# snap-research/F8Net

Hardware: AMD Instinct MI355X
Metric: images/sec at bs=128 (ResNet-50 INT8) (higher is better)
Workload: dtype int8 x int8 -> int32 (exact integer)

## Files before the change

f8net_amd/csrc/f8_cchain.hip:

```cpp
#include "f8_device.h"
#include <algorithm>
#include <cstdio>
#include <cstdlib>

namespace f8 {

struct CCfg {
    static constexpr int C = 2048, MID = 512, PXI = 49, IMG = 4, NPX = PXI * IMG, NPT = 7, G = 8;
    static constexpr int CT = C / 32, CM = MID / 32, CTC = CT / G, CMC = CM / G;
    static constexpr int NK1 = C / 32, KK = MID / 32;
    static constexpr int X8_BYTES = NPT * NK1 * 1024, M_BYTES = NPT * KK * 1024;
    static constexpr int OFF_M1 = X8_BYTES, OFF_M2 = X8_BYTES + M_BYTES, XCL_BYTES = X8_BYTES + 2 * M_BYTES;
    static constexpr int PATCH_BYTES = M_BYTES;
    static constexpr int ZERO_BYTES = 8192;
    static constexpr int D1 = 3, CH1_FR = 40, CH1_BYTES = CH1_FR * 1024;
    static constexpr int D2 = 4, CH2_BYTES = 8 * 1024;
    static constexpr int OFF_ZERO = PATCH_BYTES, OFF_RING2 = PATCH_BYTES + ZERO_BYTES;
    static constexpr int OFF_BIAS = OFF_RING2 + D2 * CH2_BYTES, BIAS_INTS = 32 * (2 * CMC + CTC);
    static constexpr int OFF_MISC = OFF_BIAS + BIAS_INTS * 4, LDS_BYTES = OFF_MISC + 256;
    static_assert(D1 * CH1_BYTES <= OFF_RING2, "the P1 ring lives in the patch's bytes (dead during P1)");
    static_assert(LDS_BYTES <= 160 * 1024, "LDS");
};
constexpr size_t kCChainXchgBytes = (size_t)32 * CCfg::XCL_BYTES;

template <int FAST>
__device__ __forceinline__ v4i cq_tile16(const v16i& y, int n, int lo, int hi, unsigned x_or) {
    unsigned d[4];
    const float sc = FAST == 1 ? requant_u8_scale(n) : 0.0f;
#pragma unroll
    for (int g = 0; g < 4; ++g) {
        if constexpr (FAST == 1) d[g] = requant_u8x4(y[4 * g], y[4 * g + 1], y[4 * g + 2], y[4 * g + 3], sc) ^ x_or;
        else if constexpr (FAST == 2) d[g] = requant_u8x4_int(y[4 * g], y[4 * g + 1], y[4 * g + 2], y[4 * g + 3], n) ^ x_or;
        else d[g] = pack4(requant1(y[4 * g], n, lo, hi), requant1(y[4 * g + 1], n, lo, hi), requant1(y[4 * g + 2], n, lo, hi), requant1(y[4 * g + 3], n, lo, hi)) ^ x_or;
    }
    auto s0 = __builtin_amdgcn_permlane32_swap(d[0], d[2], false, false);
    auto s1 = __builtin_amdgcn_permlane32_swap(d[1], d[3], false, false);
    const v4i o = {(int)s0[0], (int)s0[1], (int)s1[0], (int)s1[1]};
    return o;
}

#define F8_LDS3(p) ((__attribute__((address_space(3))) void*)(p))

#ifndef F8_CC_Q_TAIL
#define F8_CC_Q_TAIL 0
#endif
#ifndef F8_CC_Q_P1
#define F8_CC_Q_P1 0
#endif
#ifndef F8_CC_Q_P2
#define F8_CC_Q_P2 0
#endif
#ifndef F8_CC_Q_P3
#define F8_CC_Q_P3 0
#endif
#define F8_CC_QI(fast, ov) ((fast) == 1 && (ov) != 0 ? (ov) : (fast))

#ifndef F8_CC_WAR_NOPS
#define F8_CC_WAR_NOPS 16
#endif
__device__ __forceinline__ void mfma_operands_read() {
#ifdef F8_CC_NO_GUARD
    return;
#endif
    __builtin_amdgcn_sched_barrier(0);
    if constexpr (F8_CC_WAR_NOPS >= 16) asm volatile("s_nop 7\n\ts_nop 7" ::: "memory");
    else if constexpr (F8_CC_WAR_NOPS >= 8) asm volatile("s_nop 7" ::: "memory");
    else if constexpr (F8_CC_WAR_NOPS >= 4) asm volatile("s_nop 3" ::: "memory");
    else if constexpr (F8_CC_WAR_NOPS >= 2) asm volatile("s_nop 1" ::: "memory");
    else if constexpr (F8_CC_WAR_NOPS >= 1) asm volatile("s_nop 0" ::: "memory");
    __builtin_amdgcn_sched_barrier(0);
}

__device__ __forceinline__ void lds_barrier() {
    asm volatile("s_waitcnt lgkmcnt(0)" ::: "memory");
    __builtin_amdgcn_s_barrier();
    asm volatile("" ::: "memory");
}

template <int FAST>
__global__ void __launch_bounds__(512) __attribute__((amdgpu_waves_per_eu(2, 2)))
cchain_kernel(const ChainArgs a) {
    using Cfg = CCfg;
    constexpr int C = Cfg::C, NPT = Cfg::NPT, NK1 = Cfg::NK1, KK = Cfg::KK;
#ifndef F8_CC_DBG_NOSETREG
    if constexpr (FAST == 1) set_fp_round_nearest_even();
#endif
    extern __shared__ __attribute__((aligned(16))) char lds[];
    char* const ring2 = lds + Cfg::OFF_RING2;
    int* const bias_lds = (int*)(lds + Cfg::OFF_BIAS);
    int* const misc = (int*)(lds + Cfg::OFF_MISC);

    const int tid = threadIdx.x;
    const int wave = __builtin_amdgcn_readfirstlane(tid >> 6) & 7;
    const int lane = tid & 63, l31 = lane & 31, lh = lane >> 5;
    const unsigned l16 = (unsigned)(lane * 16);
    const int pp = wave & 3, kh = wave >> 2;

    if (tid == 0) misc[0] = (int)__hip_atomic_fetch_add(a.sync, 1u, __ATOMIC_RELAXED, __HIP_MEMORY_SCOPE_AGENT);
    __syncthreads();
    const int L = __builtin_amdgcn_readfirstlane(misc[0]);
    const int cl = L >> 3, c = L & 7;
    const int ncl = (int)(gridDim.x >> 3);
    const int ngroups = (a.N + Cfg::IMG - 1) / Cfg::IMG;
    const int npix = a.N * Cfg::PXI;
    unsigned* const flags = a.sync + 16;
    const unsigned long long t_limit = (unsigned long long)a.timeout_ticks;
    unsigned seq = 0;
#ifdef F8_TRACE
    unsigned tt[12] = {}; unsigned t_prev = (unsigned)__builtin_readcyclecounter();
#define F8_CT(i) do { const unsigned now_ = (unsigned)__builtin_readcyclecounter(); tt[i] += now_ - t_prev; t_prev = now_; } while (0)
#else
#define F8_CT(i)
#endif

    const __amdgpu_buffer_rsrc_t rxc = __builtin_amdgcn_make_buffer_rsrc((void*)(a.xchg + (size_t)cl * Cfg::XCL_BYTES), 0, (unsigned)Cfg::XCL_BYTES, 0x00020000);
    auto wrsrc = [](const int8_t* p) { return __builtin_amdgcn_make_buffer_rsrc((void*)p, 0, 0x7ffffff0, 0x00020000); };

    auto publish = [&]() {
        ++seq;
        asm volatile("s_waitcnt vmcnt(0)" ::: "memory");
        __syncthreads();
        if (tid == 0) __hip_atomic_store(flags + L, seq, __ATOMIC_RELAXED, __HIP_MEMORY_SCOPE_AGENT);
    };
    auto wait_all = [&]() {
        if (tid < Cfg::G && tid != c) {
            unsigned* const f = flags + cl * Cfg::G + tid;
            const unsigned long long t0 = wall_clock64();
            bool ok = true;
            while ((int)(__hip_atomic_load(f, __ATOMIC_RELAXED, __HIP_MEMORY_SCOPE_AGENT) - seq) < 0) {
                __builtin_amdgcn_s_sleep(1);
                if (wall_clock64() - t0 > t_limit) { ok = false; break; }
                if ((__hip_atomic_load(a.err, __ATOMIC_RELAXED, __HIP_MEMORY_SCOPE_AGENT) >> 8) == a.epoch) break;
            }
            if (!ok) {
                __hip_atomic_store(a.err, (a.epoch << 8) | 0x80u | ((unsigned)seq & 0x3fu), __ATOMIC_RELAXED, __HIP_MEMORY_SCOPE_AGENT);
                if (a.err_host) __hip_atomic_store(a.err_host, (a.epoch << 8) | 0x80u | ((unsigned)seq & 0x3fu), __ATOMIC_RELAXED, __HIP_MEMORY_SCOPE_SYSTEM);
            }
        }
        __syncthreads();
    };
    auto load_patch = [&](int off) {
#pragma unroll
        for (int k = 0; k < 14; ++k) {
            const int e = wave * 14 + k;
            __builtin_amdgcn_raw_ptr_buffer_load_lds(rxc, F8_LDS3(lds + e * 1024), 16, l16, off + e * 1024, 0, 17);
        }
    };

    v16i res[NPT];
    const int ct = c * Cfg::CTC + wave;

    for (int grp = cl; grp < ngroups; grp += ncl) {
        const int m0 = grp * Cfg::NPX;
        if (a.tail) {
            const ChainBlk& B = a.blk[0];
            const bool sc_first = B.res_shl == 0;
            const __amdgpu_buffer_rsrc_t rxs = __builtin_amdgcn_make_buffer_rsrc((void*)a.x8in, 0, (unsigned)(a.N * 196 * 1024), 0x00020000);
            const __amdgpu_buffer_rsrc_t rm2 = __builtin_amdgcn_make_buffer_rsrc((void*)a.m2in, 0, (unsigned)(npix * 512), 0x00020000);
            const __amdgpu_buffer_rsrc_t rwsc = wrsrc(B.wsc), rw4 = wrsrc(B.w4);
            unsigned vx, vm;
            {
                const int p = wave * 32 + l31, m = m0 + p;
                const int pi = p / Cfg::PXI, rem = p - pi * Cfg::PXI, r = rem / 7, cc = rem - r * 7;
                const bool ok = wave < NPT && p < Cfg::NPX && m < npix;
                vx = ok ? (unsigned)((((grp * Cfg::IMG + pi) * 14 + 2 * r) * 14 + 2 * cc) * 1024 + lh * 16) : kOOB;
                vm = ok ? (unsigned)(m * 512 + lh * 16) : kOOB;
            }
            auto chunk_is_sc = [&](int cq) { return sc_first ? cq < 4 : cq >= 2; };
            auto chunk_k = [&](int cq) { return sc_first ? (cq < 4 ? cq : cq - 4) : (cq < 2 ? cq : cq - 2); };
            auto issue = [&](int cq) {
                char* const buf = lds + (cq & 1) * 65536 + wave * 8192;
                const bool sc = chunk_is_sc(cq);
                const int k0 = chunk_k(cq) * 256;
#pragma unroll
                for (int st = 0; st < 8; ++st) {
                    if (sc) __builtin_amdgcn_raw_ptr_buffer_load_lds(rxs, F8_LDS3(buf + st * 1024), 16, vx, k0 + st * 32, 0, 0);
                    else __builtin_amdgcn_raw_ptr_buffer_load_lds(rm2, F8_LDS3(buf + st * 1024), 16, vm, k0 + st * 32, 0, 0);
                }
            };
            v4i wa[2][8];
            auto load_w = [&](v4i (&dst)[8], int cq) {
                const bool sc = chunk_is_sc(cq);
                const int f0 = (ct * (sc ? 32 : 16) + chunk_k(cq) * 8) * 1024;
#pragma unroll
                for (int st = 0; st < 8; ++st) dst[st] = sc ? __builtin_amdgcn_raw_buffer_load_b128(rwsc, l16, f0 + st * 1024, 0) : __builtin_amdgcn_raw_buffer_load_b128(rw4, l16, f0 + st * 1024, 0);
            };
            issue(0);
            load_w(wa[0], 0);
            {
                const int32_t* const bf = sc_first ? B.bsc : B.b4;
#pragma unroll
                for (int g = 0; g < 4; ++g) {
                    const v4i bv = *(const v4i*)(bf + ct * 32 + 8 * g + 4 * lh);
#pragma unroll
                    for (int j = 0; j < NPT; ++j)
#pragma unroll
                        for (int e = 0; e < 4; ++e) res[j][4 * g + e] = bv[e];
                }
            }
            static_for<6>([&](auto qc) {
                constexpr int Q = decltype(qc)::value;
                asm volatile("s_waitcnt vmcnt(0)" ::: "memory");
                lds_barrier();
                if constexpr (Q + 1 < 6) { issue(Q + 1); load_w(wa[(Q + 1) & 1], Q + 1); }
                const char* const buf = lds + (Q & 1) * 65536;
#pragma unroll
                for (int st = 0; st < 8; ++st)
#pragma unroll
                    for (int j = 0; j < NPT; ++j) {
                        const v4i xf = *(const v4i*)(buf + (j * 8 + st) * 1024 + l16);
                        res[j] = __builtin_amdgcn_mfma_i32_32x32x32_i8(wa[Q & 1][st], xf, res[j], 0, 0, 0);
                    }
                mfma_operands_read();
                if ((sc_first && Q == 3) || (!sc_first && Q == 1)) {
                    const int sh = sc_first ? B.acc_shl : B.res_shl;
                    const int32_t* const bs = sc_first ? B.b4 : B.bsc;
#pragma unroll
                    for (int g = 0; g < 4; ++g) {
                        const v4i bv = *(const v4i*)(bs + ct * 32 + 8 * g + 4 * lh);
#pragma unroll
                        for (int j = 0; j < NPT; ++j)
#pragma unroll
                            for (int e = 0; e < 4; ++e) res[j][4 * g + e] = (int)(((unsigned)res[j][4 * g + e] << sh) + (unsigned)bv[e]);
                    }
                }
            });
            const int floor1 = B.relu1 ? 0 : -2147483647;
            const ChainBlk& B1 = a.blk[1];
#pragma unroll
            for (int j = 0; j < NPT; ++j) {
#pragma unroll
                for (int r = 0; r < 16; ++r) res[j][r] = max(res[j][r], floor1);
                const v4i o = cq_tile16<F8_CC_QI(FAST, F8_CC_Q_TAIL)>(res[j], B1.nq, FAST ? 0 : B1.loq, FAST ? 255 : B1.hiq, FAST ? 0x80808080u : B1.xorq);
                __builtin_amdgcn_raw_buffer_store_b128(o, rxc, l16, (j * NK1 + ct) * 1024, 17);
            }
            publish();
            F8_CT(0);
        } else {
            const ChainBlk& B0 = a.blk[0];
            const __amdgpu_buffer_rsrc_t rxr = __builtin_amdgcn_make_buffer_rsrc((void*)a.xr, 0, (unsigned)(((npix + 31) & ~31) * C * 4), 0x00020000);
#pragma unroll
            for (int j = 0; j < NPT; ++j) {
                const int p = j * 32 + l31, m = m0 + p;
                const unsigned vo = (p < Cfg::NPX && m < npix) ? (unsigned)((m >> 5) * (C * 128) + lh * 512 + (m & 31) * 16) : kOOB;
#pragma unroll
                for (int g = 0; g < 4; ++g) {
                    const v4i v = __builtin_amdgcn_raw_buffer_load_b128(rxr, vo + g * 1024, ct * 4096, 0);
#pragma unroll
                    for (int e = 0; e < 4; ++e) res[j][4 * g + e] = v[e];
                }
            }
#pragma unroll
            for (int j = 0; j < NPT; ++j) {
                const v4i o = cq_tile16<FAST>(res[j], B0.nq, FAST ? 0 : B0.loq, FAST ? 255 : B0.hiq, FAST ? 0x80808080u : B0.xorq);
                __builtin_amdgcn_raw_buffer_store_b128(o, rxc, l16, (j * NK1 + ct) * 1024, 17);
            }
            publish();
            F8_CT(0);
        }

        for (int b = a.tail ? 1 : 0; b < a.nblk; ++b) {
            const ChainBlk& B = a.blk[b];
            const bool last = b + 1 == a.nblk;
            const ChainBlk& BN = a.blk[last ? b : b + 1];
            const int n1 = B.n1, n2 = B.n2, acc_shl = B.acc_shl, res_shl = B.res_shl;
            const int lo1 = FAST ? 0 : B.lo1, hi1 = FAST ? 255 : B.hi1, lo2 = FAST ? 0 : B.lo2, hi2 = FAST ? 255 : B.hi2;
            const unsigned xor1 = FAST ? 0x80808080u : B.xor1, xor2 = FAST ? 0x80808080u : B.xor2;
            const int relu_a = FAST ? 1 : B.relu_a, relu_b = FAST ? 1 : B.relu_b, relu1 = FAST ? 1 : B.relu1;
            const int nq = BN.nq, loq = FAST ? 0 : BN.loq, hiq = FAST ? 255 : BN.hiq;
            const unsigned xorq = FAST ? 0x80808080u : BN.xorq;

            {
                int bv = 0;
                if (tid < 64) bv = B.b0[c * 64 + tid];
                else if (tid < 128) bv = B.b2[c * 64 + tid - 64];
                else if (tid < Cfg::BIAS_INTS) bv = B.b4[c * 256 + tid - 128];
                if (tid < Cfg::BIAS_INTS) bias_lds[tid] = bv;
            }
            wait_all();
            F8_CT(1);

            {
                const __amdgpu_buffer_rsrc_t rw0 = wrsrc(B.w0);
                v16i acc[2][2];
#pragma unroll
                for (int jj = 0; jj < 2; ++jj)
#pragma unroll
                    for (int i = 0; i < 2; ++i)
#pragma unroll
                        for (int r = 0; r < 16; ++r) acc[jj][i][r] = 0;
                constexpr int NCH = NK1 / 4, D = Cfg::D1, NI = 5;
                auto issue = [&](int q) {
                    char* const slot = lds + (q % D) * Cfg::CH1_BYTES;
#pragma unroll
                    for (int k = 0; k < NI; ++k) {
                        const int e = wave * NI + k, t = e & 3;
                        const int step = t < 2 ? 2 * q + t : 32 + 2 * q + (t - 2);
                        if (e < 32) {
                            const int j = e >> 2;
                            __builtin_amdgcn_raw_ptr_buffer_load_lds(rxc, F8_LDS3(slot + e * 1024), 16, j < NPT ? l16 : kOOB, (j * NK1 + step) * 1024, 0, 17);
                        } else {
                            const int i = (e - 32) >> 2;
                            __builtin_amdgcn_raw_ptr_buffer_load_lds(rw0, F8_LDS3(slot + e * 1024), 16, l16, ((c * 2 + i) * NK1 + step) * 1024, 0, 0);
                        }
                    }
                };
                asm volatile("s_waitcnt vmcnt(0)" ::: "memory");
                issue(0); issue(1);
                const unsigned bb = (unsigned)((pp * 8 + kh * 2) * 1024) + l16, ab = (unsigned)((32 + kh * 2) * 1024) + l16;
                static_for<NCH>([&](auto qc) {
                    constexpr int Q = decltype(qc)::value;
                    constexpr int younger = (Q + D - 2 < NCH - 1 ? Q + D - 2 : NCH - 1) - Q;
                    wait_vmcnt<younger * NI>();
                    lds_barrier();
                    if constexpr (Q + D - 1 < NCH) issue(Q + D - 1);
                    const char* const slot = lds + (Q % D) * Cfg::CH1_BYTES;
#pragma unroll
                    for (int s = 0; s < 2; ++s) {
                        const v4i a0 = *(const v4i*)(slot + ab + s * 1024), a1 = *(const v4i*)(slot + ab + (4 + s) * 1024);
                        const v4i b0 = *(const v4i*)(slot + bb + s * 1024), b1 = *(const v4i*)(slot + bb + (4 + s) * 1024);
                        acc[0][0] = __builtin_amdgcn_mfma_i32_32x32x32_i8(a0, b0, acc[0][0], 0, 0, 0);
                        acc[0][1] = __builtin_amdgcn_mfma_i32_32x32x32_i8(a1, b0, acc[0][1], 0, 0, 0);
                        acc[1][0] = __builtin_amdgcn_mfma_i32_32x32x32_i8(a0, b1, acc[1][0], 0, 0, 0);
                        acc[1][1] = __builtin_amdgcn_mfma_i32_32x32x32_i8(a1, b1, acc[1][1], 0, 0, 0);
                    }
                });
                mfma_operands_read();
                F8_CT(2);
                __syncthreads();
#pragma unroll
                for (int jj = 0; jj < 2; ++jj)
#pragma unroll
                    for (int g = 0; g < 4; ++g) {
                        v4i o;
#pragma unroll
                        for (int e = 0; e < 4; ++e) o[e] = kh ? acc[jj][0][4 * g + e] : acc[jj][1][4 * g + e];
                        *(v4i*)(lds + (wave * 8 + jj * 4 + g) * 1024 + l16) = o;
                    }
                __syncthreads();
                const int floor0 = relu_a ? 0 : INT32_MIN;
                const int ctm = c * 2 + kh;
#pragma unroll
                for (int jj = 0; jj < 2; ++jj) {
                    v16i y;
#pragma unroll
                    for (int g = 0; g < 4; ++g) {
                        const v4i o = *(const v4i*)(lds + ((wave ^ 4) * 8 + jj * 4 + g) * 1024 + l16);
                        const v4i bv = *(const v4i*)(bias_lds + kh * 32 + 8 * g + 4 * lh);
#pragma unroll
                        for (int e = 0; e < 4; ++e) {
                            const unsigned mine = (unsigned)(kh ? acc[jj][1][4 * g + e] : acc[jj][0][4 * g + e]);
                            y[4 * g + e] = (int)(mine + (unsigned)o[e] + (unsigned)bv[e]);
                            if constexpr (!FAST) y[4 * g + e] = max(y[4 * g + e], floor0);
                        }
                    }
                    const int j = pp * 2 + jj;
                    const v4i o = cq_tile16<F8_CC_QI(FAST, F8_CC_Q_P1)>(y, n1, lo1, hi1, xor1);
                    if (j < NPT) __builtin_amdgcn_raw_buffer_store_b128(o, rxc, l16, Cfg::OFF_M1 + (j * KK + ctm) * 1024, 17);
                }
                publish();
                F8_CT(3);
            }
            {
                const v4i zv = {(int)xor1, (int)xor1, (int)xor1, (int)xor1};
                *(v4i*)(lds + Cfg::OFF_ZERO + tid * 16) = zv;
            }
            wait_all();
            F8_CT(4);

            {
                const __amdgpu_buffer_rsrc_t rw2 = wrsrc(B.w2);
                load_patch(Cfg::OFF_M1);
                constexpr int NCH = 36, D = Cfg::D2;
                auto issue = [&](int q) {
                    const int e = wave, i = e >> 2, t = e & 3;
                    const int step = (q >> 2) * KK + (t < 2 ? 0 : 8) + 2 * (q & 3) + (t & 1);
                    __builtin_amdgcn_raw_ptr_buffer_load_lds(rw2, F8_LDS3(ring2 + (q % D) * Cfg::CH2_BYTES + e * 1024), 16, l16, ((c * 2 + i) * (9 * KK) + step) * 1024, 0, 0);
                };
                issue(0); issue(1); issue(2);
                int prow[2], pcol[2];
#pragma unroll
                for (int jj = 0; jj < 2; ++jj) {
                    const int p = (pp * 2 + jj) * 32 + l31;
                    const int rem = p % Cfg::PXI, r = rem / 7;
                    prow[jj] = p < Cfg::NPX ? r : 64; pcol[jj] = rem - r * 7;
                }
                unsigned tb[2] = {0u, 0u};
                auto tap_base = [&](auto tc) {
                    constexpr int T = decltype(tc)::value, TY = T / 3 - 1, TX = T % 3 - 1;
#pragma unroll
                    for (int jj = 0; jj < 2; ++jj) {
                        const int q = (pp * 2 + jj) * 32 + l31 + TY * 7 + TX;
                        const bool ok = (unsigned)(prow[jj] + TY) < 7u && (unsigned)(pcol[jj] + TX) < 7u;
                        tb[jj] = ok ? (unsigned)((q >> 5) * (KK * 1024) + kh * 8192 + lh * 512 + (q & 31) * 16) : (unsigned)Cfg::OFF_ZERO + l16;
                    }
                };
                v16i acc[2][2];
#pragma unroll
                for (int jj = 0; jj < 2; ++jj)
#pragma unroll
                    for (int i = 0; i < 2; ++i)
#pragma unroll
                        for (int r = 0; r < 16; ++r) acc[jj][i][r] = 0;
                const unsigned ab = (unsigned)(kh * 2 * 1024) + l16;
                static_for<NCH>([&](auto qc) {
                    constexpr int Q = decltype(qc)::value, T = Q / 4;
                    constexpr int younger = (Q + D - 2 < NCH - 1 ? Q + D - 2 : NCH - 1) - Q;
                    wait_vmcnt<younger>();
                    lds_barrier();
                    if constexpr (Q + D - 1 < NCH) issue(Q + D - 1);
                    if constexpr (Q % 4 == 0) tap_base(std::integral_constant<int, T>{});
                    const char* const slot = ring2 + (Q % D) * Cfg::CH2_BYTES;
#pragma unroll
                    for (int s = 0; s < 2; ++s) {
                        const v4i a0 = *(const v4i*)(slot + ab + s * 1024), a1 = *(const v4i*)(slot + ab + (4 + s) * 1024);
                        const v4i b0 = *(const v4i*)(lds + tb[0] + (2 * (Q % 4) + s) * 1024), b1 = *(const v4i*)(lds + tb[1] + (2 * (Q % 4) + s) * 1024);
                        acc[0][0] = __builtin_amdgcn_mfma_i32_32x32x32_i8(a0, b0, acc[0][0], 0, 0, 0);
                        acc[0][1] = __builtin_amdgcn_mfma_i32_32x32x32_i8(a1, b0, acc[0][1], 0, 0, 0);
                        acc[1][0] = __builtin_amdgcn_mfma_i32_32x32x32_i8(a0, b1, acc[1][0], 0, 0, 0);
                        acc[1][1] = __builtin_amdgcn_mfma_i32_32x32x32_i8(a1, b1, acc[1][1], 0, 0, 0);
                    }
                });
                mfma_operands_read();
                F8_CT(5);
                __syncthreads();
#pragma unroll
                for (int jj = 0; jj < 2; ++jj)
#pragma unroll
                    for (int g = 0; g < 4; ++g) {
                        v4i o;
#pragma unroll
                        for (int e = 0; e < 4; ++e) o[e] = kh ? acc[jj][0][4 * g + e] : acc[jj][1][4 * g + e];
                        *(v4i*)(lds + (wave * 8 + jj * 4 + g) * 1024 + l16) = o;
                    }
                __syncthreads();
                const int floor0 = relu_b ? 0 : INT32_MIN;
                const int ctm = c * 2 + kh;
#pragma unroll
                for (int jj = 0; jj < 2; ++jj) {
                    v16i y;
#pragma unroll
                    for (int g = 0; g < 4; ++g) {
                        const v4i o = *(const v4i*)(lds + ((wave ^ 4) * 8 + jj * 4 + g) * 1024 + l16);
                        const v4i bv = *(const v4i*)(bias_lds + 64 + kh * 32 + 8 * g + 4 * lh);
#pragma unroll
                        for (int e = 0; e < 4; ++e) {
                            const unsigned mine = (unsigned)(kh ? acc[jj][1][4 * g + e] : acc[jj][0][4 * g + e]);
                            y[4 * g + e] = (int)(mine + (unsigned)o[e] + (unsigned)bv[e]);
                            if constexpr (!FAST) y[4 * g + e] = max(y[4 * g + e], floor0);
                        }
                    }
                    const int j = pp * 2 + jj;
                    const v4i o = cq_tile16<F8_CC_QI(FAST, F8_CC_Q_P2)>(y, n2, lo2, hi2, xor2);
                    if (j < NPT) __builtin_amdgcn_raw_buffer_store_b128(o, rxc, l16, Cfg::OFF_M2 + (j * KK + ctm) * 1024, 17);
                }
                publish();
                F8_CT(6);
            }

            {
                const __amdgpu_buffer_rsrc_t rw4 = wrsrc(B.w4);
                v4i wst[KK];
#pragma unroll
                for (int k = 0; k < KK; ++k) wst[k] = __builtin_amdgcn_raw_buffer_load_b128(rw4, l16, (ct * KK + k) * 1024, 0);
                v16i breg;
#pragma unroll
                for (int g = 0; g < 4; ++g) {
                    const v4i bv = *(const v4i*)(bias_lds + 128 + wave * 32 + 8 * g + 4 * lh);
#pragma unroll
                    for (int e = 0; e < 4; ++e) breg[4 * g + e] = bv[e];
                }
                wait_all();
                F8_CT(7);
                load_patch(Cfg::OFF_M2);
                asm volatile("s_waitcnt vmcnt(0)" ::: "memory");
                __syncthreads();
                F8_CT(8);
                const int floor1 = relu1 ? 0 : -2147483647;
                static_for<NPT>([&](auto jc) {
                    constexpr int J = decltype(jc)::value;
                    v16i acc;
#pragma unroll
                    for (int k = 0; k < KK; ++k) {
                        const v4i xf = *(const v4i*)(lds + (J * KK + k) * 1024 + l16);
                        if (k == 0) acc = __builtin_amdgcn_mfma_i32_32x32x32_i8(wst[k], xf, breg, 0, 0, 0);
                        else acc = __builtin_amdgcn_mfma_i32_32x32x32_i8(wst[k], xf, acc, 0, 0, 0);
                    }
                    mfma_operands_read();
                    v16i& rr = res[J];
#pragma unroll
                    for (int r = 0; r < 16; ++r) {
                        if constexpr (FAST) rr[r] = max((int)(((unsigned)acc[r] << acc_shl) + (unsigned)rr[r]), 0);
                        else rr[r] = max((int)(((unsigned)acc[r] << acc_shl) + ((unsigned)rr[r] << res_shl)), floor1);
                    }
                    if (!last) {
                        const v4i o = cq_tile16<F8_CC_QI(FAST, F8_CC_Q_P3)>(rr, nq, loq, hiq, xorq);
                        __builtin_amdgcn_raw_buffer_store_b128(o, rxc, l16, (J * NK1 + ct) * 1024, 17);
                    } else if (!a.pool) {
                        const int p = J * 32 + l31, m = m0 + p;
                        if (p < Cfg::NPX && m < npix) {
                            const unsigned tot = (unsigned)(((npix + 31) & ~31) * C);
                            if (a.out32) {
                                const __amdgpu_buffer_rsrc_t ro = __builtin_amdgcn_make_buffer_rsrc((void*)a.out32, 0, tot * 4u, 0x00020000);
                                const unsigned vo = (unsigned)((m >> 5) * (C * 128) + lh * 512 + (m & 31) * 16);
#pragma unroll
                                for (int g = 0; g < 4; ++g) {
                                    const v4i o = {rr[4 * g], rr[4 * g + 1], rr[4 * g + 2], rr[4 * g + 3]};
                                    __builtin_amdgcn_raw_buffer_store_b128(o, ro, vo + g * 1024, ct * 4096, 0);
                                }
                            }
#pragma unroll
                            for (int k = 0; k < 2; ++k)
                                if (a.q[k].ptr) {
                                    const __amdgpu_buffer_rsrc_t rq = __builtin_amdgcn_make_buffer_rsrc((void*)a.q[k].ptr, 0, tot, 0x00020000);
                                    __builtin_amdgcn_raw_buffer_store_b128(cq_tile16<0>(rr, a.q[k].n, a.q[k].lo, a.q[k].hi, a.q[k].bias_xor), rq, (unsigned)(m * C + 16 * lh), ct * 32, 0);
                                }
                        }
                    }
                });
                if (last && a.pool) {
                    const bool b0 = lane & 1, b1 = lane & 2;
                    const int n_img = grp * Cfg::IMG + (lane & 3);
#pragma unroll
                    for (int g = 0; g < 4; ++g) {
                        unsigned tot[4];
#pragma unroll
                        for (int e = 0; e < 4; ++e) {
                            unsigned sm[Cfg::IMG];
                            static_for<Cfg::IMG>([&](auto ic) {
                                constexpr int I = decltype(ic)::value, LO = I * Cfg::PXI, HI = LO + Cfg::PXI;
                                unsigned acc_i = 0;
                                static_for<NPT>([&](auto jc) {
                                    constexpr int J = decltype(jc)::value;
                                    if constexpr (J * 32 < HI && J * 32 + 32 > LO) {
                                        constexpr int L0 = LO - J * 32, L1 = HI - J * 32;
                                        acc_i += (l31 >= L0 && l31 < L1) ? (unsigned)res[J][4 * g + e] : 0u;
                                    }
                                });
                                sm[I] = acc_i;
                            });
                            const unsigned u0 = (b0 ? sm[1] : sm[0]) + (unsigned)__shfl_xor((int)(b0 ? sm[0] : sm[1]), 1);
                            const unsigned u1 = (b0 ? sm[3] : sm[2]) + (unsigned)__shfl_xor((int)(b0 ? sm[2] : sm[3]), 1);
                            unsigned v = (b1 ? u1 : u0) + (unsigned)__shfl_xor((int)(b1 ? u0 : u1), 2);
                            v += (unsigned)__shfl_xor((int)v, 4); v += (unsigned)__shfl_xor((int)v, 8); v += (unsigned)__shfl_xor((int)v, 16);
                            tot[e] = v;
                        }
                        if (l31 < Cfg::IMG && n_img < a.N) {
                            const int ch = ct * 32 + 8 * g + 4 * lh;
                            if (a.out32) { const v4i o = {(int)tot[0], (int)tot[1], (int)tot[2], (int)tot[3]}; *(v4i*)(a.out32 + i32t_index(n_img, ch, C)) = o; }
#pragma unroll
                            for (int k = 0; k < 2; ++k)
                                if (a.q[k].ptr)
                                    *(unsigned*)(a.q[k].ptr + (size_t)n_img * C + ch) =
                                        pack4(requant1((int)tot[0], a.q[k].n, a.q[k].lo, a.q[k].hi), requant1((int)tot[1], a.q[k].n, a.q[k].lo, a.q[k].hi),
                                              requant1((int)tot[2], a.q[k].n, a.q[k].lo, a.q[k].hi), requant1((int)tot[3], a.q[k].n, a.q[k].lo, a.q[k].hi)) ^ a.q[k].bias_xor;
                        }
                    }
                }
                F8_CT(9);
                if (!last) publish();
                else __syncthreads();
                F8_CT(10);
            }
        }
    }
    if (tid == 0) {
        asm volatile("s_waitcnt vmcnt(0)" ::: "memory");
        misc[2] = (__hip_atomic_fetch_add(a.sync + 1, 1u, __ATOMIC_RELAXED, __HIP_MEMORY_SCOPE_AGENT) == gridDim.x - 1u) ? 1 : 0;
    }
    __syncthreads();
    if (misc[2]) {
        for (int i = tid; i < (int)gridDim.x; i += 512) __hip_atomic_store(flags + i, 0u, __ATOMIC_RELAXED, __HIP_MEMORY_SCOPE_AGENT);
        if (tid == 0) { __hip_atomic_store(a.sync, 0u, __ATOMIC_RELAXED, __HIP_MEMORY_SCOPE_AGENT); __hip_atomic_store(a.sync + 1, 0u, __ATOMIC_RELAXED, __HIP_MEMORY_SCOPE_AGENT); }
    }
#ifdef F8_TRACE
    if (a.trace && lane == 0) {
        unsigned* tp = (unsigned*)a.trace + ((size_t)blockIdx.x * 8 + wave) * 16;
        for (int i = 0; i < 12; ++i) tp[i] = tt[i];
        tp[12] = (unsigned)L;
    }
#endif
}

bool cchain_supported(int C, int MID, int H, int W, int cin0, bool tail) { return C == 2048 && MID == 512 && H == 7 && W == 7 && cin0 == (tail ? 1024 : 2048); }
size_t cchain_xchg_bytes() { return kCChainXchgBytes; }
int cchain_clusters(int N, int slots) {
    const int groups = (N + CCfg::IMG - 1) / CCfg::IMG, cap = std::min(slots / CCfg::G, 32);
    if (cap < 1) return 0;
    const int rounds = (groups + cap - 1) / cap;
    return (groups + rounds - 1) / rounds;
}
int cchain_kernel_name(char* buf, size_t cap, int fast) { return snprintf(buf, cap, "f8::cchain_kernel<%d>", fast != 0 ? 2 : 0); }

template <int FAST>
static hipError_t launch_cchain_t(const ChainArgs& a, hipStream_t s) {
    static unsigned long long attr_done = 0; int attr_dev = -1;
    if (!dyn_lds_opted_in(&attr_done, &attr_dev)) {
        hipError_t e = hipFuncSetAttribute((const void*)cchain_kernel<FAST>, hipFuncAttributeMaxDynamicSharedMemorySize, CCfg::LDS_BYTES);
        if (e != hipSuccess) return e;
        if (attr_dev >= 0) attr_done |= 1ull << attr_dev;
    }
    const int grid = a.NG * CCfg::G;
    if (a.NG < 1 || grid > 256 || (a.tail ? (!a.x8in || !a.m2in || a.nblk < 2) : !a.xr)) return hipErrorInvalidValue;
#ifdef F8_TRACE
    static unsigned* tbuf = nullptr; static int count = 0;
    static const int want = [] { const char* e = getenv("F8_TRACE_CHAIN7"); return e ? atoi(e) : -1; }();
    ChainArgs b = a;
    const bool tracing = (count++ == want);
    if (tracing) { if (!tbuf) (void)hipMalloc((void**)&tbuf, (size_t)256 * 8 * 64); (void)hipMemsetAsync(tbuf, 0, (size_t)grid * 8 * 64, s); b.trace = tbuf; }
    hipLaunchKernelGGL((cchain_kernel<FAST>), dim3(grid), dim3(512), CCfg::LDS_BYTES, s, b);
    if (tracing) {
        (void)hipStreamSynchronize(s);
        static unsigned hb[256 * 8 * 16];
        (void)hipMemcpy(hb, tbuf, (size_t)grid * 8 * 64, hipMemcpyDeviceToHost);
        static const char* nm[11] = {"stage-in+publish", "wait x8", "P1 loop", "P1 epilogue+publish", "wait mid1", "P2 loop", "P2 epilogue+publish", "wait mid2", "P3 patch load", "P3 compute", "P3 publish"};
        for (int w : {0, 3, 4, 7}) {
            double ph[12] = {};
            for (int i = 0; i < grid; ++i) for (int k = 0; k < 12; ++k) ph[k] += (double)hb[((size_t)i * 8 + w) * 16 + k];
            fprintf(stderr, "[trace cchain<%d>] grid %d, %d blocks, N %d, wave %d: avg cycles per WG (whole launch):", FAST, grid, a.nblk, a.N, w);
            double tot = 0;
            for (int k = 0; k < 11; ++k) { fprintf(stderr, " %s %.0f |", nm[k], ph[k] / grid); tot += ph[k] / grid; }
            fprintf(stderr, " total %.0f\n", tot);
        }
    }
#else
    hipLaunchKernelGGL((cchain_kernel<FAST>), dim3(grid), dim3(512), CCfg::LDS_BYTES, s, a);
#endif
    return hipGetLastError();
}

hipError_t launch_cchain(const ChainArgs& a, int fast, hipStream_t s) {
#ifdef F8_CC_FLOAT_INSTANCE
    if (fast == 1) return launch_cchain_t<1>(a, s);
#endif
    return fast != 0 ? launch_cchain_t<2>(a, s) : launch_cchain_t<0>(a, s);
}

}
```

Measured before the change: 156,800.

## Deepen tail-phase LDS ring to four smaller chunks with two-ahead prefetch

The tail (downsample+conv3) phase now splits its K loop into 12 chunks of 128 instead of 6 chunks of 256. It uses a 4-deep LDS ring, issues loads two chunks ahead and waits with a partial vmcnt instead of draining all loads each step. Separately, lane and offset values are rematerialised per phase behind opaque asm barriers. This stops the compiler hoisting them into long-lived registers and keeps scalar offset bases out of VGPRs, easing register pressure. The cost is more barriers per tail and more LDS use, plus reliance on an exact vmcnt count.

```diff
diff --git a/f8net_amd/csrc/f8_cchain.hip b/f8net_amd/csrc/f8_cchain.hip
--- a/f8net_amd/csrc/f8_cchain.hip
+++ b/f8net_amd/csrc/f8_cchain.hip
@@ -15,10 +15,12 @@
     static constexpr int ZERO_BYTES = 8192;
     static constexpr int D1 = 3, CH1_FR = 40, CH1_BYTES = CH1_FR * 1024;
     static constexpr int D2 = 4, CH2_BYTES = 8 * 1024;
+    static constexpr int DT = 4, NCHT = 12, CHT_BYTES = 32 * 1024;
     static constexpr int OFF_ZERO = PATCH_BYTES, OFF_RING2 = PATCH_BYTES + ZERO_BYTES;
     static constexpr int OFF_BIAS = OFF_RING2 + D2 * CH2_BYTES, BIAS_INTS = 32 * (2 * CMC + CTC);
     static constexpr int OFF_MISC = OFF_BIAS + BIAS_INTS * 4, LDS_BYTES = OFF_MISC + 256;
     static_assert(D1 * CH1_BYTES <= OFF_RING2, "the P1 ring lives in the patch's bytes (dead during P1)");
+    static_assert(DT * CHT_BYTES <= OFF_BIAS, "the TAIL ring lives below the biases (everything else is dead during the TAIL)");
     static_assert(LDS_BYTES <= 160 * 1024, "LDS");
 };
 constexpr size_t kCChainXchgBytes = (size_t)32 * CCfg::XCL_BYTES;
@@ -41,6 +43,8 @@
 
 #define F8_LDS3(p) ((__attribute__((address_space(3))) void*)(p))
 
+__device__ __forceinline__ int cc_opaque(int v) { asm volatile("" : "+s"(v)); return v; }
+
 #ifndef F8_CC_Q_TAIL
 #define F8_CC_Q_TAIL 0
 #endif
@@ -92,8 +96,11 @@
 
     const int tid = threadIdx.x;
     const int wave = __builtin_amdgcn_readfirstlane(tid >> 6) & 7;
-    const int lane = tid & 63, l31 = lane & 31, lh = lane >> 5;
-    const unsigned l16 = (unsigned)(lane * 16);
+#define CC_LANES                                                                                                                        \
+    int tq_ = tid; asm volatile("" : "+v"(tq_));                                                                                        \
+    const int lane = tq_ & 63, l31 = lane & 31, lh = lane >> 5;                                                                         \
+    const unsigned l16 = (unsigned)(lane * 16);                                                                                         \
+    (void)l31; (void)lh; (void)l16
     const int pp = wave & 3, kh = wave >> 2;
 
     if (tid == 0) misc[0] = (int)__hip_atomic_fetch_add(a.sync, 1u, __ATOMIC_RELAXED, __HIP_MEMORY_SCOPE_AGENT);
@@ -140,10 +147,11 @@
         __syncthreads();
     };
     auto load_patch = [&](int off) {
+        CC_LANES;
 #pragma unroll
         for (int k = 0; k < 14; ++k) {
             const int e = wave * 14 + k;
-            __builtin_amdgcn_raw_ptr_buffer_load_lds(rxc, F8_LDS3(lds + e * 1024), 16, l16, off + e * 1024, 0, 17);
+            __builtin_amdgcn_raw_ptr_buffer_load_lds(rxc, F8_LDS3(lds + e * 1024), 16, l16, cc_opaque(off + wave * 14 * 1024) + k * 1024, 0, 17);
         }
     };
 
@@ -153,6 +161,7 @@
     for (int grp = cl; grp < ngroups; grp += ncl) {
         const int m0 = grp * Cfg::NPX;
         if (a.tail) {
+            CC_LANES;
             const ChainBlk& B = a.blk[0];
             const bool sc_first = B.res_shl == 0;
             const __amdgpu_buffer_rsrc_t rxs = __builtin_amdgcn_make_buffer_rsrc((void*)a.x8in, 0, (unsigned)(a.N * 196 * 1024), 0x00020000);
@@ -166,27 +175,29 @@
                 vx = ok ? (unsigned)((((grp * Cfg::IMG + pi) * 14 + 2 * r) * 14 + 2 * cc) * 1024 + lh * 16) : kOOB;
                 vm = ok ? (unsigned)(m * 512 + lh * 16) : kOOB;
             }
-            auto chunk_is_sc = [&](int cq) { return sc_first ? cq < 4 : cq >= 2; };
-            auto chunk_k = [&](int cq) { return sc_first ? (cq < 4 ? cq : cq - 4) : (cq < 2 ? cq : cq - 2); };
-            auto issue = [&](int cq) {
-                char* const buf = lds + (cq & 1) * 65536 + wave * 8192;
-                const bool sc = chunk_is_sc(cq);
-                const int k0 = chunk_k(cq) * 256;
-#pragma unroll
-                for (int st = 0; st < 8; ++st) {
-                    if (sc) __builtin_amdgcn_raw_ptr_buffer_load_lds(rxs, F8_LDS3(buf + st * 1024), 16, vx, k0 + st * 32, 0, 0);
-                    else __builtin_amdgcn_raw_ptr_buffer_load_lds(rm2, F8_LDS3(buf + st * 1024), 16, vm, k0 + st * 32, 0, 0);
-                }
+            const int n1 = sc_first ? 8 : 4;
+            auto chunk_sc = [&](int q) { return (q < cc_opaque(n1)) == sc_first; };
+            auto chunk_k = [&](int q) { const int n = cc_opaque(n1); return q < n ? q : q - n; };
+            auto issue = [&](int q) {
+                char* const buf = lds + (q & 3) * Cfg::CHT_BYTES + wave * 4096;
+                const bool sc = chunk_sc(q);
+                const __amdgpu_buffer_rsrc_t r = sc ? rxs : rm2;
+                const unsigned v = sc ? vx : vm;
+                const int k0 = chunk_k(q) * 128;
+#pragma unroll
+                for (int st = 0; st < 4; ++st) __builtin_amdgcn_raw_ptr_buffer_load_lds(r, F8_LDS3(buf + st * 1024), 16, v, k0 + st * 32, 0, 0);
             };
-            v4i wa[2][8];
-            auto load_w = [&](v4i (&dst)[8], int cq) {
-                const bool sc = chunk_is_sc(cq);
-                const int f0 = (ct * (sc ? 32 : 16) + chunk_k(cq) * 8) * 1024;
-#pragma unroll
-                for (int st = 0; st < 8; ++st) dst[st] = sc ? __builtin_amdgcn_raw_buffer_load_b128(rwsc, l16, f0 + st * 1024, 0) : __builtin_amdgcn_raw_buffer_load_b128(rw4, l16, f0 + st * 1024, 0);
+            v4i wa[2][4];
+            auto load_w = [&](v4i (&dst)[4], int q) {
+                const bool sc = chunk_sc(q);
+                const __amdgpu_buffer_rsrc_t r = sc ? rwsc : rw4;
+                const int f0 = cc_opaque((ct * (sc ? 32 : 16) + chunk_k(q) * 4) * 1024);
+#pragma unroll
+                for (int st = 0; st < 4; ++st) dst[st] = __builtin_amdgcn_raw_buffer_load_b128(r, l16, f0 + st * 1024, 0);
             };
-            issue(0);
+            asm volatile("s_waitcnt vmcnt(0)" ::: "memory");
             load_w(wa[0], 0);
+            issue(0); issue(1);
             {
                 const int32_t* const bf = sc_first ? B.bsc : B.b4;
 #pragma unroll
@@ -198,33 +209,38 @@
                         for (int e = 0; e < 4; ++e) res[j][4 * g + e] = bv[e];
                 }
             }
-            static_for<6>([&](auto qc) {
+            static_for<Cfg::NCHT>([&](auto qc) {
                 constexpr int Q = decltype(qc)::value;
-                asm volatile("s_waitcnt vmcnt(0)" ::: "memory");
+                if constexpr (Q + 1 < Cfg::NCHT) wait_vmcnt<4>();
+                else wait_vmcnt<0>();
                 lds_barrier();
-                if constexpr (Q + 1 < 6) { issue(Q + 1); load_w(wa[(Q + 1) & 1], Q + 1); }
-                const char* const buf = lds + (Q & 1) * 65536;
-#pragma unroll
-                for (int st = 0; st < 8; ++st)
+                if constexpr (Q + 1 < Cfg::NCHT) load_w(wa[(Q + 1) & 1], Q + 1);
+                if constexpr (Q + 2 < Cfg::NCHT) issue(Q + 2);
+                const char* const buf = lds + (Q & 3) * Cfg::CHT_BYTES;
+#pragma unroll
+                for (int st = 0; st < 4; ++st)
 #pragma unroll
                     for (int j = 0; j < NPT; ++j) {
-                        const v4i xf = *(const v4i*)(buf + (j * 8 + st) * 1024 + l16);
+                        const v4i xf = *(const v4i*)(buf + (j * 4 + st) * 1024 + l16);
                         res[j] = __builtin_amdgcn_mfma_i32_32x32x32_i8(wa[Q & 1][st], xf, res[j], 0, 0, 0);
                     }
-                mfma_operands_read();
-                if ((sc_first && Q == 3) || (!sc_first && Q == 1)) {
-                    const int sh = sc_first ? B.acc_shl : B.res_shl;
-                    const int32_t* const bs = sc_first ? B.b4 : B.bsc;
-#pragma unroll
-                    for (int g = 0; g < 4; ++g) {
-                        const v4i bv = *(const v4i*)(bs + ct * 32 + 8 * g + 4 * lh);
-#pragma unroll
-                        for (int j = 0; j < NPT; ++j)
-#pragma unroll
-                            for (int e = 0; e < 4; ++e) res[j][4 * g + e] = (int)(((unsigned)res[j][4 * g + e] << sh) + (unsigned)bv[e]);
+                if constexpr (Q == 3 || Q == 7) {
+                    mfma_operands_read();
+                    if (Q + 1 == n1) {
+                        const int sh = sc_first ? B.acc_shl : B.res_shl;
+                        const int32_t* const bs = sc_first ? B.b4 : B.bsc;
+#pragma unroll
+                        for (int g = 0; g < 4; ++g) {
+                            const v4i bv = *(const v4i*)(bs + ct * 32 + 8 * g + 4 * lh);
+#pragma unroll
+                            for (int j = 0; j < NPT; ++j)
+#pragma unroll
+                                for (int e = 0; e < 4; ++e) res[j][4 * g + e] = (int)(((unsigned)res[j][4 * g + e] << sh) + (unsigned)bv[e]);
+                        }
                     }
                 }
             });
+            mfma_operands_read();
             const int floor1 = B.relu1 ? 0 : -2147483647;
             const ChainBlk& B1 = a.blk[1];
 #pragma unroll
@@ -237,6 +253,7 @@
             publish();
             F8_CT(0);
         } else {
+            CC_LANES;
             const ChainBlk& B0 = a.blk[0];
             const __amdgpu_buffer_rsrc_t rxr = __builtin_amdgcn_make_buffer_rsrc((void*)a.xr, 0, (unsigned)(((npix + 31) & ~31) * C * 4), 0x00020000);
 #pragma unroll
@@ -281,6 +298,7 @@
             F8_CT(1);
 
             {
+                CC_LANES;
                 const __amdgpu_buffer_rsrc_t rw0 = wrsrc(B.w0);
                 v16i acc[2][2];
 #pragma unroll
@@ -301,7 +319,7 @@
                             __builtin_amdgcn_raw_ptr_buffer_load_lds(rxc, F8_LDS3(slot + e * 1024), 16, j < NPT ? l16 : kOOB, (j * NK1 + step) * 1024, 0, 17);
                         } else {
                             const int i = (e - 32) >> 2;
-                            __builtin_amdgcn_raw_ptr_buffer_load_lds(rw0, F8_LDS3(slot + e * 1024), 16, l16, ((c * 2 + i) * NK1 + step) * 1024, 0, 0);
+                            __builtin_amdgcn_raw_ptr_buffer_load_lds(rw0, F8_LDS3(slot + e * 1024), 16, l16, cc_opaque(c * 2 * NK1 * 1024) + (i * NK1 + step) * 1024, 0, 0);
                         }
                     }
                 };
@@ -369,13 +387,14 @@
             F8_CT(4);
 
             {
+                CC_LANES;
                 const __amdgpu_buffer_rsrc_t rw2 = wrsrc(B.w2);
                 load_patch(Cfg::OFF_M1);
                 constexpr int NCH = 36, D = Cfg::D2;
                 auto issue = [&](int q) {
                     const int e = wave, i = e >> 2, t = e & 3;
                     const int step = (q >> 2) * KK + (t < 2 ? 0 : 8) + 2 * (q & 3) + (t & 1);
-                    __builtin_amdgcn_raw_ptr_buffer_load_lds(rw2, F8_LDS3(ring2 + (q % D) * Cfg::CH2_BYTES + e * 1024), 16, l16, ((c * 2 + i) * (9 * KK) + step) * 1024, 0, 0);
+                    __builtin_amdgcn_raw_ptr_buffer_load_lds(rw2, F8_LDS3(ring2 + (q % D) * Cfg::CH2_BYTES + e * 1024), 16, l16, cc_opaque(c * 2 * 9 * KK * 1024) + (i * (9 * KK) + step) * 1024, 0, 0);
                 };
                 issue(0); issue(1); issue(2);
                 int prow[2], pcol[2];
@@ -459,10 +478,11 @@
             }
 
             {
+                CC_LANES;
                 const __amdgpu_buffer_rsrc_t rw4 = wrsrc(B.w4);
                 v4i wst[KK];
 #pragma unroll
-                for (int k = 0; k < KK; ++k) wst[k] = __builtin_amdgcn_raw_buffer_load_b128(rw4, l16, (ct * KK + k) * 1024, 0);
+                for (int k = 0; k < KK; ++k) wst[k] = __builtin_amdgcn_raw_buffer_load_b128(rw4, l16, cc_opaque(ct * KK * 1024) + k * 1024, 0);
                 v16i breg;
 #pragma unroll
                 for (int g = 0; g < 4; ++g) {
@@ -574,7 +594,7 @@
         if (tid == 0) { __hip_atomic_store(a.sync, 0u, __ATOMIC_RELAXED, __HIP_MEMORY_SCOPE_AGENT); __hip_atomic_store(a.sync + 1, 0u, __ATOMIC_RELAXED, __HIP_MEMORY_SCOPE_AGENT); }
     }
 #ifdef F8_TRACE
-    if (a.trace && lane == 0) {
+    if (a.trace && (tid & 63) == 0) {
         unsigned* tp = (unsigned*)a.trace + ((size_t)blockIdx.x * 8 + wave) * 16;
         for (int i = 0; i < 12; ++i) tp[i] = tt[i];
         tp[12] = (unsigned)L;
```

Result: faster. 159,700 (median of 6 runs) (+1.9%).
